# 011235813/discrete_mean_field_game

Hardware: AMD Instinct MI355X
Metric: env-steps/sec for batched d-bin population rollouts (higher is better)
Workload: dtype f32 (f64 accumulate); 1 GPU; actor_critic.train(update_every="rollout") of the drop-in class (mfg_ac2.train call surface; device-side start draw every episode, one update per 15-step rollout): d=21 topics, T=15, global batch 65536 = 65536 trajectories per GPU x 1; d=21, T=15, batch_per_gpu=65536, global_batch=65536, rng=philox4x32-10, parallelism=trajectory-sharded x1, 1 all-reduce/update

## Files before the change

### discrete_mean_field_game_amd/_lib.py

```python
from __future__ import annotations

import ctypes as C
import os
import subprocess

_HERE = os.path.dirname(os.path.abspath(__file__))
CSRC = os.path.join(_HERE, 'csrc')
LIB_PATH = os.environ.get('MFG_HIP_LIB') or os.path.join(CSRC, 'libmfg_hip.so')

MFG_MAX_D = 512
REWARD_MFG_AC2, REWARD_SYNTHETIC, REWARD_EXTERNAL = 0, 1, 2
ROLLOUT_WRITE_P, ROLLOUT_TD, ROLLOUT_DISCOUNT_POW, ROLLOUT_F64, TRAIN_APPLY = 1, 2, 4, 8, 16
PRECISION_F64, PRECISION_MIXED = 0, 1
POP_MAX_K = 65535
POP_RESIDENT_MAX_TILES = 64
STATUS_MIXED_RANGE = 1
STATUS_POP_NONFINITE = 2
ECOMM = -6
RN_TRAIN_MAX_TRAJ = 64
FORECAST_MAX_RANKS = 8
FORECAST_MAX_REPEATS = 1024
PRECISIONS = {'f64': PRECISION_F64, 'mixed': PRECISION_MIXED, 0: 0, 1: 1}


class MfgError(RuntimeError):
    code = 0


def build(force: bool = False) -> str:
    args = ['make', '-C', CSRC]
    if force:
        args.append('-B')
    subprocess.run(args, check=True, stdout=subprocess.PIPE, stderr=subprocess.STDOUT)
    return LIB_PATH


_p = C.c_void_p
_i64, _i32, _u64, _u32, _f64, _sz = C.c_int64, C.c_int, C.c_uint64, C.c_uint32, C.c_double, C.c_size_t

SIGNATURES = {
    'mfg_last_error': (C.c_char_p, []),
    'mfg_abi_version': (_i32, []),
    'mfg_set_core_mapping': (_i32, [_i32]),
    'mfg_init': (_i32, []),
    'mfg_status': (_i32, [C.POINTER(C.c_uint)]),
    'mfg_clear_status': (_i32, []),
    'mfg_ctx_create': (_i32, [C.POINTER(C.c_void_p)]),
    'mfg_ctx_destroy': (_i32, [_p]),
    'mfg_ctx_bind': (_i32, [_p]),
    'mfg_ctx_current': (_p, []),
    'mfg_ctx_status': (_i32, [_p, C.POINTER(C.c_uint)]),
    'mfg_ctx_clear_status': (_i32, [_p]),
    'mfg_ctx_adopt_comm': (_i32, [_p, _p]),
    'mfg_ctx_comm': (_p, [_p]),
    'mfg_device_info': (_i32, [C.POINTER(C.c_int), C.c_char_p, _i32]),
    'mfg_feature_index': (_i64, [_i32, _i32, _i32]),
    'mfg_num_features': (_i64, [_i32]),
    'mfg_workspace_bytes': (_sz, [_i64, _i32]),
    'mfg_gather_start': (_i32, [_p, _i64, _p, _i64, _i32, _p, _p]),
    'mfg_draw_start': (_i32, [_p, _i64, _i64, _i32, _u64, _u32, _u64, _p, _p, _p]),
    'mfg_alpha': (_i32, [_p, _i64, _i32, _p, _f64, _p, _p, _p]),
    'mfg_dirichlet_from_gamma': (_i32, [_p, _i64, _i32, _p, _p]),
    'mfg_sample_dirichlet': (_i32, [_p, _i64, _i32, _p, _f64, _f64, _u64, _u32, _u64, _i32, _p, _p]),
    'mfg_philox_raw': (_i32, [_u64, _u32, _u32, _u32, _u32, _i64, _p, _p]),
    'mfg_step_given_P': (_i32, [_p, _p, _i64, _i32, _i32, _p, _p, _p]),
    'mfg_value': (_i32, [_p, _p, _i64, _i32, _p, _p]),
    'mfg_features': (_i32, [_p, _i64, _i32, _p, _p]),
    'mfg_score': (_i32, [_p, _p, _i64, _i32, _p, _f64, _i32, _p, _p]),
    'mfg_td_pg_accumulate': (_i32, [_p, _p, _p, _p, _p, _p, _f64, _f64, _i64, _i32, _i32, _p, _p, _p, _i32, _p, _sz,
                                   _p]),
    'mfg_apply_update': (_i32, [_p, _i32, _f64, _f64, _p, _p, _p, _p]),
    'mfg_rollout': (_i32, [_p, _i64, _i32, _i32, _p, _f64, _f64, _p, _f64, _i32, _u64, _u32, _u64, _i32,
                           _p, _p, _p, _p, _p, _p, _p, _i32, _p, _sz, _p]),
    'mfg_jsd': (_i32, [_p, _p, _i64, _i32, _p, _p]),
    'mfg_grad_accumulate': (_i32, [_p, _i64, _p, _p, _p, _i64, _i32, _i32, _i32, _p, _i32, _p, _sz, _p]),
    'mfg_grad_apply': (_i32, [_p, _i64, _p, _p, _p, _i64, _i32, _i32, _i32, _p, _f64, _f64, _p, _p, _p, _p, _sz, _p]),
# ... 124 lines not shown
```

### discrete_mean_field_game_amd/csrc/mfg_grad.h

```cpp
#pragma once
#include <hip/hip_runtime.h>
#include <stdint.h>

#include "mfg_core.h"

using namespace mfg;

constexpr int MFG_GRAD_SMALL_MAX_D = 28;
constexpr int GR_OUT_PER_THREAD = 4;
constexpr int GR_OUT_PER_BLOCK = GR_OUT_PER_THREAD * BLOCK;

struct GradArgs {
  const float* pi;
  int64_t stride_b;
  const double* delta;
  const double* g;
  const float* reward;
  int64_t N;
  int T, d, chunk;
  int64_t nsb;
  double* partial;
  int add_reward;
  unsigned* counter;
  double* G;
  int accumulate, apply;
  double lr_c, lr_a;
  double *w, *theta, *reward_acc;
};

__device__ __forceinline__ void grad_partial_body(const GradArgs& a) {
  extern __shared__ __attribute__((aligned(16))) unsigned char smem_raw[];
  const int d = a.d, Q = d * (d + 1) / 2, F = Q + d + 1, FO = F + 3;
  double* dl = reinterpret_cast<double*>(smem_raw);
  float* sp = reinterpret_cast<float*>(dl + 3 * a.chunk);
  const int tid = threadIdx.x;
// ... 47 lines not shown
      } else if (kind[u] == 2) {
        for (int q = 0; q < cn; ++q) s_ += dl[3 * q];
      } else if (kind[u] == 3) {
        for (int q = 0; q < cn; ++q) s_ += dl[3 * q + 1];
      } else if (kind[u] == 4) {
        for (int q = 0; q < cn; ++q) s_ += dl[3 * q + 2];
      } else if (kind[u] == 5) {
        s_ += (double)cn;
      }
      acc[u] = s_;
    }
  }
#pragma unroll
  for (int u = 0; u < GR_OUT_PER_THREAD; ++u) {
    const int k = blockIdx.y * GR_OUT_PER_BLOCK + u * BLOCK + tid;
    if (kind[u] >= 0) a.partial[(int64_t)blockIdx.x * FO + k] = acc[u];
  }
}
#ifndef MFG_GRAD_BODIES_ONLY
__global__ __launch_bounds__(BLOCK) void k_grad_partial(GradArgs a) { grad_partial_body(a); }
#endif

#ifndef MFG_GRAD_BODIES_ONLY
__global__ void k_add_reward(double* __restrict__ delta, const float* __restrict__ reward, int64_t N) {
  for (int64_t n = blockIdx.x * (int64_t)blockDim.x + threadIdx.x; n < N; n += (int64_t)gridDim.x * blockDim.x)
    delta[n] += (double)reward[n];
}
#endif

constexpr int GS_CH = 64;
#ifndef MFG_GS_BPC
#define MFG_GS_BPC 2
#endif

template <int D>
struct GradChunk {
  static constexpr int NL = D ? D : MFG_GRAD_SMALL_MAX_D;
  float pi[NL];
  double de, dg;
  float rr;
};

template <int D, bool WIDE>
__device__ __forceinline__ void grad_chunk_load(GradChunk<D>& c, const GradArgs& a, const double* gp, const float* rp, int d,
                                                int64_t n0, int64_t b0, int s0, int lane, float invT, float inv_d) {
  const int last = (int)((a.N - 1 - n0) < (GS_CH - 1) ? (a.N - 1 - n0) : (GS_CH - 1));
  {
    const int64_t n = n0 + (lane < last ? lane : last);
    c.de = a.delta[n];
    c.dg = gp[n];
    c.rr = rp[n];
  }
  if constexpr (!WIDE) {
    const float* cb = a.pi + b0 * a.stride_b + (int64_t)s0 * d;
    const int extra = (int)(a.stride_b - (int64_t)a.T * d);
#pragma unroll
    for (int k = 0; k < GradChunk<D>::NL; ++k) {
      if (!D && k * WAVE >= GS_CH * d) {
        c.pi[k] = 0.0f;
        continue;
      }
      int e = k * WAVE + lane;
      int j = (int)(((float)e + 0.5f) * inv_d);
      if (j > last) { j = last; e = last * d; }
      const int q = (int)(((float)(s0 + j) + 0.5f) * invT);
      c.pi[k] = cb[(unsigned)(e + __mul24(q, extra))];
// ... 104 lines not shown
  __syncthreads();
  double (*red)[3][4][WAVE] = reinterpret_cast<double (*)[3][4][WAVE]>(smem);
#pragma unroll
  for (int v = 0; v < 4; ++v) {
    red[wv][0][v][lane] = c00[v];
    red[wv][1][v][lane] = c01[v];
    red[wv][2][v][lane] = c11[v];
  }
  __syncthreads();
  double* out = a.partial + (int64_t)blockIdx.x * FO;
  for (int e = tid; e < 3 * 4 * WAVE; e += BLOCK) {
    const int t = e / (4 * WAVE), v = (e / WAVE) & 3, l = e & (WAVE - 1);
    const int gi = (t == 2 ? 16 : 0) + 4 * v + (l >> 4), gj = (t == 0 ? 0 : 16) + (l & 15);
    int k = -1;
    if (gj < d) {
      if (gi <= gj) k = feat_idx(gi, gj, d);
    } else if (gj == d) {
      if (gi <= d) k = Q + gi;
    } else if (gj == d + 1) {
      if (gi == d) k = F;
    } else if (gj == d + 2) {
      if (gi == d + 1) k = F + 1;
    } else if (gj == d + 3) {
      if (gi == d + 1) k = F + 2;
    }
    if (k >= 0) {
      double tsum = red[0][t][v][l];
#pragma unroll
      for (int q = 1; q < WAVES; ++q) tsum += red[q][t][v][l];
      out[k] = tsum;
    }
  }
  if (!a.counter) return;
  __shared__ int s_last;
  __threadfence();
  __syncthreads();
  if (tid == 0) s_last = (atomicAdd(a.counter, 1u) == gridDim.x - 1) ? 1 : 0;
  __syncthreads();
  if (!s_last) return;
  __threadfence();
  double* fin = &red[0][0][0][0];
  const int nrows = (int)gridDim.x;
  for (int k = tid; k < FO; k += BLOCK) {
    double s0 = 0.0, s1 = 0.0, s2 = 0.0, s3 = 0.0;
    const double* col = a.partial + k;
    int r = 0;
    for (; r + 7 < nrows; r += 8) {
      const double v0 = col[(int64_t)r * FO], v1 = col[(int64_t)(r + 1) * FO], v2 = col[(int64_t)(r + 2) * FO],
                   v3 = col[(int64_t)(r + 3) * FO], v4 = col[(int64_t)(r + 4) * FO], v5 = col[(int64_t)(r + 5) * FO],
                   v6 = col[(int64_t)(r + 6) * FO], v7 = col[(int64_t)(r + 7) * FO];
      s0 += v0;
      s1 += v1;
      s2 += v2;
      s3 += v3;
      s0 += v4;
      s1 += v5;
      s2 += v6;
      s3 += v7;
    }
    for (; r < nrows; ++r) s0 += col[(int64_t)r * FO];
    const double tot = (s0 + s1) + (s2 + s3);
    const double gk = a.accumulate ? a.G[k] + tot : tot;
    a.G[k] = gk;
    fin[k] = gk;
  }
  __syncthreads();
  if (a.apply) {
    const double count = fin[F + 2];
    if (count > 0.0) {
      const double inv = 1.0 / count;
      for (int k = tid; k < F; k += BLOCK) a.w[k] = updated_param(a.w[k], a.lr_c, fin[k], inv);
      if (tid == 0) {
        if (a.reward_acc) *a.reward_acc += fin[F + 1] * inv;
        *a.theta = updated_param(*a.theta, a.lr_a, fin[F], inv);
      }
    }
  }
  if (tid == 0) *a.counter = 0u;
}
template <int D, bool WIDE = false>
__global__ __launch_bounds__(BLOCK) void k_grad_mfma_small(GradArgs a) { grad_mfma_small_body<D, WIDE>(a); }

constexpr int GM_KC = 32;
#ifndef MFG_GM_TPW
#define MFG_GM_TPW 8
#endif
constexpr int GM_TPW = MFG_GM_TPW;

template <int NPF>
__device__ __forceinline__ void grad_mfma_body(const GradArgs& a, int tpw) {
  extern __shared__ __attribute__((aligned(16))) unsigned char smem_raw[];
  const int d = a.d, nt = d >> 4, pitch = d + 16;
  const int Q = d * (d + 1) / 2, F = Q + d + 1, FO = F + 3;
  double* dl = reinterpret_cast<double*>(smem_raw);
  double* red = dl + GM_KC;
  float* sp = reinterpret_cast<float*>(red + 4 * BLOCK);
  const int tid = threadIdx.x, lane = tid & (WAVE - 1), wv = tid / WAVE;
  const int ntiles = nt * (nt + 1) / 2;
  const int t0 = ((int)blockIdx.y * WAVES + wv) * tpw;
  int nmine = ntiles - t0;
  nmine = nmine < 0 ? 0 : (nmine > tpw ? tpw : nmine);
  int tr[GM_TPW], tc[GM_TPW];
#pragma unroll
  for (int i = 0; i < GM_TPW; ++i) {
    int t = t0 + i, r = 0;
    if (i < nmine) {
      while (t >= nt - r) {
        t -= nt - r;
        ++r;
      }
    } else {
      t = 0;
    }
    tr[i] = r;
// ... 233 lines not shown
```

### discrete_mean_field_game_amd/csrc/mfg_kernels.hip

```cpp
#include <hip/hip_runtime.h>
#include <stdarg.h>
#include <stdint.h>
#include <stdio.h>
#include <string.h>
#include <stdlib.h>

#include <dlfcn.h>

#include <atomic>
#include <mutex>
#include <unordered_map>

#include "../../include/mfg_hip.h"
#include "mfg_core.h"
#include "mfg_evaluate_pop.h"
#include "mfg_forecast_pop.h"
#include "mfg_irl_population.h"
#include "mfg_population.h"

using namespace mfg;

static thread_local char g_err[512] = "";

static int fail(int code, const char* fmt, ...) {
// ... 1383 lines not shown

struct ApplyArgs {
  double lr_c, lr_a;
  double *w, *theta, *reward_acc;
};
static void launch_apply_update(const double* G, int d, double lr_c, double lr_a, double* w, double* theta, double* reward_acc,
                                hipStream_t st) {
  const int64_t F = mfg_num_features(d);
  hipLaunchKernelGGL(k_apply_update, dim3((unsigned)((F + 255) / 256)), dim3(256), 0, st, G, F, lr_c, lr_a, w, theta, reward_acc);
}

static bool value_batch_ok(int d) { return d > WAVE && d % 16 == 0 && d <= MFG_MAX_D; }
static size_t value_buffer_bytes(int64_t N, int d) { return value_batch_ok(d) ? (size_t)(2 * N) * 8 : 0; }

static void grad_geometry(int64_t N, int d, int* chunk, int64_t* nsb, int* nob) {
  const int64_t FO = mfg_num_features(d) + 3;
  int ch = 8192 / d;
  if (ch > 64) ch = 64;
  if (ch < 8) ch = 8;
  *chunk = ch;
  int64_t sb = (N + ch - 1) / ch;
#ifndef MFG_GRAD_WS_MB
#define MFG_GRAD_WS_MB 72
#endif
  int64_t cap = (int64_t)((long long)MFG_GRAD_WS_MB << 20) / (FO * 8);
  if (cap > 1024) cap = 1024;
  if (cap < 16) cap = 16;
  if (sb > cap) sb = cap;
  if (sb < 1) sb = 1;
  *nsb = sb;
  *nob = (int)((FO + GR_OUT_PER_BLOCK - 1) / GR_OUT_PER_BLOCK);
}

static int launch_grad(const float* pi, int64_t stride_b, const double* delta, const double* g, const float* reward,
                       int64_t N, int T, int d, double* G, int accumulate, void* ws, size_t ws_bytes, hipStream_t st,
                       const ApplyArgs* apply = nullptr, bool* applied = nullptr, bool add_reward = false,
                       const PopArgs* pop = nullptr) {
  if (applied) *applied = false;
  const int64_t FO = mfg_num_features(d) + 3;
  int chunk, nob;
  int64_t nsb;
  grad_geometry(N, d, &chunk, &nsb, &nob);
  const size_t need = (size_t)(nsb * FO * 8) + MFG_WS_CONTROL_BYTES;
  if (ws_bytes < need) return fail(MFG_EWORKSPACE, "%s: need %lld bytes, have %lld", "workspace", (long long)need,
                                   (long long)ws_bytes);
  ReduceApply rap{};
  if (apply && !accumulate) {
    rap.on = 1;
    rap.lr_c = apply->lr_c;
    rap.lr_a = apply->lr_a;
    rap.count = (double)N;
    rap.w = apply->w;
    rap.theta = apply->theta;
    rap.reward_acc = apply->reward_acc;
  }
  GradArgs a{};
  a.pi = pi;
  a.stride_b = stride_b;
  a.delta = delta;
  a.g = g;
  a.reward = reward;
  a.N = N;
  a.T = T;
  a.d = d;
  a.chunk = chunk;
  a.nsb = nsb;
  a.partial = reinterpret_cast<double*>((char*)ws + MFG_WS_CONTROL_BYTES);
  const bool small = d <= MFG_GRAD_SMALL_MAX_D;
  if (add_reward && !small)
    hipLaunchKernelGGL(k_add_reward, dim3(grid_for(N, 256, 8)), dim3(256), 0, st, const_cast<double*>(delta), reward, N);
  if (small) {
    a.add_reward = add_reward ? 1 : 0;
    const int64_t NC = (N + GS_CH - 1) / GS_CH;
    int64_t blocks = (NC + WAVES - 1) / WAVES;
    const int64_t cap = (int64_t)num_cus() * MFG_GS_BPC;
    if (blocks > cap) blocks = cap;
    if (blocks > nsb) blocks = nsb;
    if (blocks < 1) blocks = 1;
    a.nsb = blocks;
    const bool fuse = blocks <= MFG_GRAD_FUSE_MAX_ROWS;
    if (fuse) {
      a.counter = reinterpret_cast<unsigned*>(ws);
      a.G = G;
      a.accumulate = accumulate;
      if (apply) {
        a.apply = 1;
        a.lr_c = apply->lr_c;
        a.lr_a = apply->lr_a;
        a.w = apply->w;
        a.theta = apply->theta;
        a.reward_acc = apply->reward_acc;
        if (applied) *applied = true;
      }
    }
    const bool wide = stride_b - (int64_t)T * d >= (1 << 23);
    if (pop) {
      if (wide) return fail(MFG_EUNSUPPORTED, "%s", "population: trajectory stride beyond the small gradient kernel");
      launch_grad_mfma_small_pop(d == 21 || d == 15 ? d : 0, (unsigned)blocks, a, *pop, st);
      if (fuse) return check_launch("grad_mfma_small_pop");
      launch_reduce_partials_pop((unsigned)((FO + RP_OUT - 1) / RP_OUT), (const double*)a.partial, blocks, FO, G, rap, *pop, st);
      if (applied && rap.on) *applied = true;
      return check_launch("grad_mfma_small_pop");
    }
    if (wide) hipLaunchKernelGGL((k_grad_mfma_small<0, true>), dim3((unsigned)blocks), dim3(BLOCK), 0, st, a);
    else if (d == 21) hipLaunchKernelGGL((k_grad_mfma_small<21>), dim3((unsigned)blocks), dim3(BLOCK), 0, st, a);
    else if (d == 15) hipLaunchKernelGGL((k_grad_mfma_small<15>), dim3((unsigned)blocks), dim3(BLOCK), 0, st, a);
    else hipLaunchKernelGGL((k_grad_mfma_small<0>), dim3((unsigned)blocks), dim3(BLOCK), 0, st, a);
    if (fuse) return check_launch("grad_mfma_small");
    hipLaunchKernelGGL(k_reduce_partials, dim3((unsigned)((FO + RP_OUT - 1) / RP_OUT)), dim3(RP_SLICES * RP_OUT), 0, st,
                       (const double*)a.partial, blocks, FO, accumulate, G, rap);
    if (applied && rap.on) *applied = true;
    return check_launch("grad_mfma_small");
  }
  if (d % 16 == 0 && d >= 64 && d <= 4 * BLOCK) {
    const int nt = d / 16, ntiles = nt * (nt + 1) / 2;
    const int ny = (ntiles + WAVES * GM_TPW - 1) / (WAVES * GM_TPW);
    const int tpw = (ntiles + ny * WAVES - 1) / (ny * WAVES);
    a.chunk = (BLOCK % (d / 4) == 0 && (((uintptr_t)pi & 15) == 0) && (stride_b % 4 == 0)) ? 1 : 0;
    const size_t lds_m = (size_t)GM_KC * 8 + (size_t)4 * BLOCK * 8 + (size_t)GM_KC * (d + 16) * 4;
    const int npf = a.chunk ? d / 32 : 0;
    if (pop) {
      if (npf != 0 && npf != 2) return fail(MFG_EUNSUPPORTED, "%s", "population: d > 64");
      launch_grad_mfma_pop(npf, (unsigned)nsb, (unsigned)ny, lds_m, a, tpw, *pop, st);
      launch_reduce_partials_pop((unsigned)((FO + RP_OUT - 1) / RP_OUT), (const double*)a.partial, nsb, FO, G, rap, *pop, st);
      if (applied && rap.on) *applied = true;
      return check_launch("grad_mfma_pop");
    }
#ifndef MFG_GRAD_MFMA_OLD
    if (a.chunk && (d == 128 || d == 256)) {
#ifndef MFG_GM2_BPC128
#define MFG_GM2_BPC128 3
#endif
      const int64_t want = d == 256 ? (int64_t)num_cus() * 2 / Gm2Geom<256>::NY : (int64_t)num_cus() * MFG_GM2_BPC128 / Gm2Geom<128>::NY;
      if (nsb > want) nsb = want;
      a.nsb = nsb;
      if (d == 256) hipLaunchKernelGGL((k_grad_mfma2<256>), dim3((unsigned)nsb, (unsigned)Gm2Geom<256>::NY), dim3(BLOCK), lds_m, st, a);
      else hipLaunchKernelGGL((k_grad_mfma2<128>), dim3((unsigned)nsb, (unsigned)Gm2Geom<128>::NY), dim3(BLOCK), lds_m, st, a);
// ... 179 lines not shown
  ReduceApply rap{};
  if (apply && !accumulate) {
    rap.on = 1;
    rap.lr_c = apply->lr_c;
    rap.lr_a = apply->lr_a;
    rap.count = (double)B;
    rap.w = apply->w;
    rap.theta = apply->theta;
    rap.reward_acc = apply->reward_acc;
  }
  if (pop) {
    if (accumulate) return fail(MFG_EUNSUPPORTED, "%s", "population: accumulated sums");
    launch_reduce_partials_pop((unsigned)((FO + RP_OUT - 1) / RP_OUT), (const double*)((char*)ws + MFG_WS_CONTROL_BYTES), nt, FO, G,
                               rap, *pop, st);
    return check_launch("core_sums_pop");
  }
  hipLaunchKernelGGL(k_reduce_partials, dim3((unsigned)((FO + RP_OUT - 1) / RP_OUT)), dim3(RP_SLICES * RP_OUT), 0, st,
                     (const double*)((char*)ws + MFG_WS_CONTROL_BYTES), nt, FO, accumulate, G, rap);
  return check_launch("core_sums");
}

extern "C" {

const char* mfg_last_error(void) { return g_err; }
int mfg_abi_version(void) { return 18; }

int mfg_init(void) {
  if (!htab_ptr()) return fail(MFG_ELAUNCH, "%s", "mfg_init: no HIP device / table initialisation failed");
  if (!status_word().host) return fail(MFG_ELAUNCH, "%s", "mfg_init: status word allocation failed");
  return MFG_OK;
}

int mfg_set_core_mapping(int mode) { return core_mapping_set(mode); }

int mfg_status(unsigned* bits_host) {
  const StatusWord sw = status_word();
  if (!sw.host) return fail(MFG_ELAUNCH, "%s", "status word allocation failed");
  const unsigned bits = *(volatile unsigned*)sw.host;
  if (bits_host) *bits_host = bits;
  return bits ? status_error(bits) : MFG_OK;
}

int mfg_clear_status(void) {
  const StatusWord sw = status_word();
  if (!sw.host) return fail(MFG_ELAUNCH, "%s", "status word allocation failed");
  *(volatile unsigned*)sw.host = 0u;
  return MFG_OK;
}

int mfg_ctx_create(mfg_ctx_t** ctx_out) {
  REQUIRE(ctx_out, "null pointer");
  int dev = 0;
  if (hipGetDevice(&dev) != hipSuccess || dev < 0 || dev >= 64) return fail(MFG_ELAUNCH, "%s", "mfg_ctx_create: no HIP device");
  if (!htab_ptr()) return fail(MFG_ELAUNCH, "%s", "mfg_ctx_create: table initialisation failed");
  mfg_ctx* c = new (std::nothrow) mfg_ctx();
  if (!c) return fail(MFG_ELAUNCH, "%s", "mfg_ctx_create: out of memory");
  c->device = dev;
  if (!alloc_status_word(&c->sw)) {
    delete c;
    return fail(MFG_ELAUNCH, "%s", "mfg_ctx_create: status word allocation failed");
  }
  {
    std::lock_guard<std::mutex> lock(g_ctx_mu);
    g_ctx_live[c] = g_ctx_next_gen++;
  }
  *ctx_out = c;
// ... 1674 lines not shown
```

### discrete_mean_field_game_amd/csrc/mfg_population.h

```cpp
#pragma once
#include <hip/hip_runtime.h>
#include <stdint.h>

#include "mfg_core.h"

struct GradArgs;
struct ReduceApply;

namespace mfg {

struct PopArgs {
  int K;
  int L;
  int64_t F;
  int64_t s_pi0;
  int64_t s_gpi;
  int64_t s_traj;
  int64_t s_state;
  int64_t s_n;
  int64_t s_acc;
  int64_t s_ws;
  const uint64_t* seed;
  const double *shift, *alpha_scale, *lr_c, *lr_a;
  double sc, sa;
  int64_t s_P;
  int64_t s_theta_b;
  int64_t N;
  int64_t s_idx;
  int32_t* idx;
  const int32_t* state;
  unsigned* status;
};

__device__ __forceinline__ bool pop_retired(const PopArgs& p, int k) { return p.state[k] != 0; }

template <class P>
__device__ __forceinline__ P* pop_at(P* p, int64_t stride, int k) {
  return p ? p + stride * k : p;
}
template <class P>
__device__ __forceinline__ P* pop_bytes(P* p, int64_t bytes, int k) {
  using C = std::conditional_t<std::is_const_v<P>, const char, char>;
  return p ? reinterpret_cast<P*>(reinterpret_cast<C*>(p) + bytes * k) : p;
}

template <bool SUMS, int STEP, bool CTL = false>
__device__ __forceinline__ CoreArgs pop_core_args(const CoreArgs& a, const PopArgs& p, int k) {
  CoreArgs b = a;
  b.pi0 = pop_at(a.pi0, p.s_pi0, k);
  if constexpr (STEP == 0) b.theta = a.theta + k;
  else b.theta = pop_bytes(a.theta, p.s_theta_b, k);
  b.w = pop_at(a.w, p.F, k);
  b.shift = p.shift[k];
  b.alpha_scale = p.alpha_scale[k];
  b.seed = p.seed[k];
  if constexpr (CTL) b.status = p.status + k;
  b.pi_traj = pop_at(a.pi_traj, p.s_traj, k);
  b.pi_next_out = pop_at(a.pi_next_out, p.s_state, k);
  if constexpr (STEP == 0) b.reward_out = pop_at(a.reward_out, p.s_n, k);
  b.delta = pop_at(a.delta, p.s_n, k);
  b.g = pop_at(a.g, p.s_n, k);
  if constexpr (!SUMS) b.P_out = pop_at(a.P_out, p.s_P, k);
  if constexpr (SUMS) b.part_rows = pop_bytes(a.part_rows, p.s_ws, k);
  if constexpr (STEP == 2) b.pi_start_out = pop_at(a.pi_start_out, p.s_state, k);
  if constexpr (STEP == 1) {
    b.step_G = pop_at(a.step_G, p.F + 3, k);
    b.step_rows = pop_bytes(a.step_rows, p.s_ws, k);
    b.w_out = pop_at(a.w_out, p.F, k);
    b.theta_out = pop_bytes(a.theta_out, p.s_ws, k);
    b.pend_reward_acc = pop_at(a.pend_reward_acc, p.s_acc, k);
    b.pend_lr_c = p.lr_c[k] * p.sc;
    b.pend_lr_a = p.lr_a[k] * p.sa;
  }
  return b;
}

int launch_core_pop(const CoreArgs& a, const PopArgs& p, bool fast, int num_cus, hipStream_t st);
int launch_eval_rollout_pop(const CoreArgs& a, const PopArgs& p, bool fast, int num_cus, hipStream_t st);
void launch_draw_start_pop(int grid, const float* mat, int64_t num_start, int64_t B, int d, uint32_t step, uint64_t traj_offset,
                           float* out, const PopArgs& p, hipStream_t st);
void launch_grad_mfma_small_pop(int D, unsigned blocks, const GradArgs& a, const PopArgs& p, hipStream_t st);
void launch_grad_partial_pop(unsigned nsb, unsigned nob, size_t lds, const GradArgs& a, const PopArgs& p, hipStream_t st);
void launch_grad_mfma_pop(int npf, unsigned nsb, unsigned ny, size_t lds, const GradArgs& a, int tpw, const PopArgs& p,
                          hipStream_t st);
void launch_reduce_partials_pop(unsigned nob, const double* partial, int64_t nsb, int64_t FO, double* G, const ReduceApply& ap,
                                const PopArgs& p, hipStream_t st);
void launch_reduce_rows_apply_pop(const double* rows, int nrows, int64_t FO, double* G, double count, double* w,
                                  const double* theta_in, double* theta_out, double* reward_acc, const PopArgs& p, hipStream_t st);

struct PopResidentArgs {
  const float* mat_pi0;
  int64_t num_start;
  float *pi_io, *pi_scratch;
  double *theta, *w, *G;
  double* reward_acc;
  int T, episodes;
  uint32_t first_step;
  double sc[MFG_POP_RESIDENT_EPISODES], sa[MFG_POP_RESIDENT_EPISODES];
};
int launch_pop_resident(const CoreArgs& a, const PopArgs& p, const PopResidentArgs& r, bool fast, hipStream_t st);

void launch_pop_retire(const mfg_pop_control_t& c, const double* theta, const double* w, int64_t F, const double* shift, bool mixed,
                       bool after_episode, hipStream_t st);

}
```

### discrete_mean_field_game_amd/csrc/mfg_population.hip

```cpp
#include "mfg_core.h"
#define MFG_GRAD_BODIES_ONLY
#include "mfg_grad.h"
#include "mfg_population.h"

namespace mfg {

#define MFG_CORE_POP_BOUNDS __launch_bounds__(BLOCK, SUMS ? 2 : (FAST ? MFG_CORE_SMALL_WAVES : MFG_CORE_SMALL_WAVES_F64))
template <bool FAST, int D, bool SUMS, int STEP>
__global__ MFG_CORE_POP_BOUNDS void k_core_pop(CoreArgs a, PopArgs p) {
  core_small_body<true, true, FAST, D, SUMS, STEP>(pop_core_args<SUMS, STEP>(a, p, blockIdx.y));
}
template <bool FAST, int D, bool SUMS, int STEP>
__global__ MFG_CORE_POP_BOUNDS void k_core_pop_ctl(CoreArgs a, PopArgs p) {
  if (pop_retired(p, blockIdx.y)) return;
  core_small_body<true, true, FAST, D, SUMS, STEP>(pop_core_args<SUMS, STEP, true>(a, p, blockIdx.y));
}
#undef MFG_CORE_POP_BOUNDS

template <bool FAST, int D, bool SUMS, int STEP>
static void go_pop(const CoreArgs& a, const PopArgs& p, int num_cus, size_t lds, hipStream_t st) {
  const int red = STEP == 1 ? core_step_red_blocks(a.d * (a.d + 1) / 2 + a.d + 1 + 3) : 0;
  if (p.state) {
    const int grid = core_small_grid<k_core_pop_ctl<FAST, D, SUMS, STEP>>(a, lds, num_cus) + red;
    hipLaunchKernelGGL((k_core_pop_ctl<FAST, D, SUMS, STEP>), dim3((unsigned)grid, (unsigned)p.K), dim3(BLOCK), lds, st, a, p);
// ... 25 lines not shown
  if (fast) go_pop<true, D, false, 0>(a, p, num_cus, lds, st);
  else go_pop<false, D, false, 0>(a, p, num_cus, lds, st);
}

int launch_core_pop(const CoreArgs& a, const PopArgs& p, bool fast, int num_cus, hipStream_t st) {
  const int d = a.d;
  if (d > WAVE) return MFG_EUNSUPPORTED;
  const size_t lds = core_small_lds(d, a.w != nullptr, true);
  if (d == 21) dispatch_pop<21>(a, p, fast, num_cus, lds, st);
  else if (d == 15) dispatch_pop<15>(a, p, fast, num_cus, lds, st);
  else if (!a.part_rows && a.step_nrows == 0) dispatch_pop<0>(a, p, fast, num_cus, lds, st);
  else return MFG_EUNSUPPORTED;
  return MFG_OK;
}

__global__ void k_draw_start_pop(const float* __restrict__ mat, int64_t num_start, int64_t B, int d, uint32_t step,
                                 uint64_t traj_offset, float* __restrict__ out, PopArgs p) {
  const int k = blockIdx.y;
  draw_start_body(mat, num_start, B, d, p.seed[k], step, traj_offset, nullptr, out + p.s_state * k);
}
__global__ void k_draw_start_pop_ctl(const float* __restrict__ mat, int64_t num_start, int64_t B, int d, uint32_t step,
                                     uint64_t traj_offset, float* __restrict__ out, PopArgs p) {
  const int k = blockIdx.y;
  if (pop_retired(p, k)) return;
  draw_start_body(mat, num_start, B, d, p.seed[k], step, traj_offset, nullptr, out + p.s_state * k);
}

void launch_draw_start_pop(int grid, const float* mat, int64_t num_start, int64_t B, int d, uint32_t step, uint64_t traj_offset,
                           float* out, const PopArgs& p, hipStream_t st) {
  hipLaunchKernelGGL(p.state ? k_draw_start_pop_ctl : k_draw_start_pop, dim3((unsigned)grid, (unsigned)p.K), dim3(256), 0, st, mat,
                     num_start, B, d, step, traj_offset, out, p);
}

__device__ __forceinline__ void pop_rebase_grad(GradArgs& a, const PopArgs& p, int k) {
  a.pi += p.s_gpi * k;
  a.delta += p.s_n * k;
  a.g += p.s_n * k;
  a.reward = pop_at(a.reward, p.s_n, k);
  a.partial = pop_bytes(a.partial, p.s_ws, k);
  a.counter = pop_bytes(a.counter, p.s_ws, k);
  a.G = pop_at(a.G, p.F + 3, k);
  a.w = pop_at(a.w, p.F, k);
  a.theta = pop_at(a.theta, 1, k);
  a.reward_acc = pop_at(a.reward_acc, p.s_acc, k);
  a.lr_c = p.lr_c[k] * p.sc;
  a.lr_a = p.lr_a[k] * p.sa;
}

template <int D>
__global__ __launch_bounds__(BLOCK) void k_grad_mfma_small_pop(GradArgs a, PopArgs p) {
  GradArgs b = a;
  pop_rebase_grad(b, p, blockIdx.y);
  grad_mfma_small_body<D, false>(b);
}
template <int D>
__global__ __launch_bounds__(BLOCK) void k_grad_mfma_small_pop_ctl(GradArgs a, PopArgs p) {
  if (pop_retired(p, blockIdx.y)) return;
  GradArgs b = a;
  pop_rebase_grad(b, p, blockIdx.y);
  grad_mfma_small_body<D, false>(b);
}

__global__ __launch_bounds__(BLOCK) void k_grad_partial_pop(GradArgs a, PopArgs p) {
  GradArgs b = a;
  pop_rebase_grad(b, p, blockIdx.z);
  grad_partial_body(b);
}
__global__ __launch_bounds__(BLOCK) void k_grad_partial_pop_ctl(GradArgs a, PopArgs p) {
  if (pop_retired(p, blockIdx.z)) return;
  GradArgs b = a;
  pop_rebase_grad(b, p, blockIdx.z);
  grad_partial_body(b);
}

template <int NPF>
__global__ __launch_bounds__(BLOCK) void k_grad_mfma_pop(GradArgs a, int tpw, PopArgs p) {
  GradArgs b = a;
  pop_rebase_grad(b, p, blockIdx.z);
  grad_mfma_body<NPF>(b, tpw);
}
template <int NPF>
// ... 119 lines not shown
```

### include/mfg_hip.h

```cpp
#ifndef MFG_HIP_H
#define MFG_HIP_H

#include <stddef.h>
#include <stdint.h>

#ifdef __cplusplus
extern "C" {
#endif

typedef void* mfg_stream_t;

enum {
  MFG_OK = 0,
  MFG_EINVAL = -1,
  MFG_ELAUNCH = -2,
  MFG_EUNSUPPORTED = -3,
  MFG_EWORKSPACE = -4,
  MFG_ERANGE = -5,
  MFG_ECOMM = -6
};

#define MFG_MAX_D 512

#define MFG_TRAJ_ID_LIMIT (1ull << 48)

enum {
  MFG_REWARD_MFG_AC2 = 0,
  MFG_REWARD_SYNTHETIC = 1,
  MFG_REWARD_EXTERNAL = 2
};

enum { MFG_PRECISION_F64 = 0, MFG_PRECISION_MIXED = 1 };

enum {
  MFG_ROLLOUT_WRITE_P = 1,
  MFG_ROLLOUT_TD = 2,
  MFG_ROLLOUT_DISCOUNT_POW = 4,
  MFG_ROLLOUT_F64 = 8
};

const char* mfg_last_error(void);
int mfg_abi_version(void);

int mfg_set_core_mapping(int mode);

int mfg_init(void);

enum { MFG_STATUS_MIXED_RANGE = 1,
       MFG_STATUS_POP_NONFINITE = 2  };
int mfg_status(unsigned* bits_host);
int mfg_clear_status(void);

typedef struct mfg_ctx mfg_ctx_t;
int mfg_ctx_create(mfg_ctx_t** ctx_out);
int mfg_ctx_destroy(mfg_ctx_t* ctx);
int mfg_ctx_bind(mfg_ctx_t* ctx);
mfg_ctx_t* mfg_ctx_current(void);
int mfg_ctx_status(mfg_ctx_t* ctx, unsigned* bits_host);
int mfg_ctx_clear_status(mfg_ctx_t* ctx);
int mfg_ctx_adopt_comm(mfg_ctx_t* ctx, void* comm);
void* mfg_ctx_comm(mfg_ctx_t* ctx);

typedef struct mfg_pop_control {
  int32_t* state;
  unsigned* status;
  double* theta_prev;
  int32_t* episodes_run;
  const double* stop_criteria;
  int32_t K;
} mfg_pop_control_t;
int mfg_ctx_set_pop_control(mfg_ctx_t* ctx, const mfg_pop_control_t* block);

int mfg_device_info(int* cu_count_host, char* arch_host, int arch_len);

int64_t mfg_feature_index(int i, int j, int d);
int64_t mfg_num_features(int d);

// ... 260 lines not shown
```

Baseline: 1.058 billion env-steps/s.

## Add lane-per-sample gradient kernel with per-wave output roles for d=15/21

Adds a new small-d gradient kernel that gives each lane one sample of a 64-sample chunk. Output features are split across the four waves, so each wave accumulates its share of the quadratic/linear features in f64 registers instead of using the MFMA tile path. Chunks are double-buffered through LDS with a prefetch stage, and the finishing reduction is factored into a shared helper. The new kernel is selected when N is at least 245760; here N = 65536 × 15 = 983040, so it runs by default. Risks include higher register and LDS pressure, and scalar f64 FMAs replacing matrix-core work.

```diff
diff --git a/discrete_mean_field_game_amd/_lib.py b/discrete_mean_field_game_amd/_lib.py
--- a/discrete_mean_field_game_amd/_lib.py
+++ b/discrete_mean_field_game_amd/_lib.py
@@ -42,6 +42,8 @@
     'mfg_last_error': (C.c_char_p, []),
     'mfg_abi_version': (_i32, []),
     'mfg_set_core_mapping': (_i32, [_i32]),
+    'mfg_set_grad_kernel': (_i32, [_i32]),
+    'mfg_grad_lane_table': (_i32, [_i32, _i32, _p, _p, _p, _i32]),
     'mfg_init': (_i32, []),
     'mfg_status': (_i32, [C.POINTER(C.c_uint)]),
     'mfg_clear_status': (_i32, []),
diff --git a/discrete_mean_field_game_amd/csrc/mfg_grad.h b/discrete_mean_field_game_amd/csrc/mfg_grad.h
--- a/discrete_mean_field_game_amd/csrc/mfg_grad.h
+++ b/discrete_mean_field_game_amd/csrc/mfg_grad.h
@@ -1,6 +1,8 @@
 #pragma once
 #include <hip/hip_runtime.h>
 #include <stdint.h>
+
+#include <utility>
 
 #include "mfg_core.h"
 
@@ -114,6 +116,54 @@
 #ifndef MFG_GS_BPC
 #define MFG_GS_BPC 2
 #endif
+
+__device__ __forceinline__ void grad_small_finish(const GradArgs& a, double* fin, int F, int FO) {
+  const int tid = threadIdx.x;
+  __shared__ int s_last;
+  __threadfence();
+  __syncthreads();
+  if (tid == 0) s_last = (atomicAdd(a.counter, 1u) == gridDim.x - 1) ? 1 : 0;
+  __syncthreads();
+  if (!s_last) return;
+  __threadfence();
+  const int nrows = (int)gridDim.x;
+  for (int k = tid; k < FO; k += BLOCK) {
+    double s0 = 0.0, s1 = 0.0, s2 = 0.0, s3 = 0.0;
+    const double* col = a.partial + k;
+    int r = 0;
+    for (; r + 7 < nrows; r += 8) {
+      const double v0 = col[(int64_t)r * FO], v1 = col[(int64_t)(r + 1) * FO], v2 = col[(int64_t)(r + 2) * FO],
+                   v3 = col[(int64_t)(r + 3) * FO], v4 = col[(int64_t)(r + 4) * FO], v5 = col[(int64_t)(r + 5) * FO],
+                   v6 = col[(int64_t)(r + 6) * FO], v7 = col[(int64_t)(r + 7) * FO];
+      s0 += v0;
+      s1 += v1;
+      s2 += v2;
+      s3 += v3;
+      s0 += v4;
+      s1 += v5;
+      s2 += v6;
+      s3 += v7;
+    }
+    for (; r < nrows; ++r) s0 += col[(int64_t)r * FO];
+    const double tot = (s0 + s1) + (s2 + s3);
+    const double gk = a.accumulate ? a.G[k] + tot : tot;
+    a.G[k] = gk;
+    fin[k] = gk;
+  }
+  __syncthreads();
+  if (a.apply) {
+    const double count = fin[F + 2];
+    if (count > 0.0) {
+      const double inv = 1.0 / count;
+      for (int k = tid; k < F; k += BLOCK) a.w[k] = updated_param(a.w[k], a.lr_c, fin[k], inv);
+      if (tid == 0) {
+        if (a.reward_acc) *a.reward_acc += fin[F + 1] * inv;
+        *a.theta = updated_param(*a.theta, a.lr_a, fin[F], inv);
+      }
+    }
+  }
+  if (tid == 0) *a.counter = 0u;
+}
 
 template <int D>
 struct GradChunk {
@@ -284,54 +334,204 @@
     }
   }
   if (!a.counter) return;
-  __shared__ int s_last;
-  __threadfence();
-  __syncthreads();
-  if (tid == 0) s_last = (atomicAdd(a.counter, 1u) == gridDim.x - 1) ? 1 : 0;
-  __syncthreads();
-  if (!s_last) return;
-  __threadfence();
-  double* fin = &red[0][0][0][0];
-  const int nrows = (int)gridDim.x;
-  for (int k = tid; k < FO; k += BLOCK) {
-    double s0 = 0.0, s1 = 0.0, s2 = 0.0, s3 = 0.0;
-    const double* col = a.partial + k;
-    int r = 0;
-    for (; r + 7 < nrows; r += 8) {
-      const double v0 = col[(int64_t)r * FO], v1 = col[(int64_t)(r + 1) * FO], v2 = col[(int64_t)(r + 2) * FO],
-                   v3 = col[(int64_t)(r + 3) * FO], v4 = col[(int64_t)(r + 4) * FO], v5 = col[(int64_t)(r + 5) * FO],
-                   v6 = col[(int64_t)(r + 6) * FO], v7 = col[(int64_t)(r + 7) * FO];
-      s0 += v0;
-      s1 += v1;
-      s2 += v2;
-      s3 += v3;
-      s0 += v4;
-      s1 += v5;
-      s2 += v6;
-      s3 += v7;
-    }
-    for (; r < nrows; ++r) s0 += col[(int64_t)r * FO];
-    const double tot = (s0 + s1) + (s2 + s3);
-    const double gk = a.accumulate ? a.G[k] + tot : tot;
-    a.G[k] = gk;
-    fin[k] = gk;
-  }
-  __syncthreads();
-  if (a.apply) {
-    const double count = fin[F + 2];
-    if (count > 0.0) {
-      const double inv = 1.0 / count;
-      for (int k = tid; k < F; k += BLOCK) a.w[k] = updated_param(a.w[k], a.lr_c, fin[k], inv);
-      if (tid == 0) {
-        if (a.reward_acc) *a.reward_acc += fin[F + 1] * inv;
-        *a.theta = updated_param(*a.theta, a.lr_a, fin[F], inv);
-      }
-    }
-  }
-  if (tid == 0) *a.counter = 0u;
+  grad_small_finish(a, &red[0][0][0][0], F, FO);
 }
 template <int D, bool WIDE = false>
 __global__ __launch_bounds__(BLOCK) void k_grad_mfma_small(GradArgs a) { grad_mfma_small_body<D, WIDE>(a); }
+
+constexpr int GL_ROLES = WAVES;
+#ifndef MFG_GL_PF
+#define MFG_GL_PF 1
+#endif
+constexpr int GL_PF = MFG_GL_PF;
+constexpr int GL_RED_ACC = 16;
+__host__ __device__ constexpr int grad_lane_fo(int d) { return d * (d + 1) / 2 + d + 1 + 3; }
+__host__ __device__ constexpr int grad_lane_role_start(int d, int r) {
+  return r * (grad_lane_fo(d) / GL_ROLES) + (r < grad_lane_fo(d) % GL_ROLES ? r : grad_lane_fo(d) % GL_ROLES);
+}
+__host__ __device__ constexpr int grad_lane_role_count(int d, int r) {
+  return grad_lane_role_start(d, r + 1) - grad_lane_role_start(d, r);
+}
+__host__ __device__ constexpr int grad_lane_row_start(int d, int i) { return i * d - (i * (i - 1)) / 2; }
+__host__ __device__ constexpr int grad_lane_out_kind(int d, int k) {
+  const int Q = d * (d + 1) / 2;
+  return k < Q ? 0 : (k < Q + d ? 1 : 2 + (k - (Q + d)));
+}
+__host__ __device__ constexpr int grad_lane_out_row(int d, int k) {
+  const int Q = d * (d + 1) / 2;
+  if (k >= Q) return k < Q + d ? k - Q : 0;
+  int i = 0;
+  while (i + 1 < d && grad_lane_row_start(d, i + 1) <= k) ++i;
+  return i;
+}
+__host__ __device__ constexpr int grad_lane_out_col(int d, int k) {
+  const int Q = d * (d + 1) / 2;
+  if (k >= Q) return 0;
+  const int i = grad_lane_out_row(d, k);
+  return i + (k - grad_lane_row_start(d, i));
+}
+
+template <int D, int K>
+__device__ __forceinline__ void grad_lane_one(double& acc, const double (&p)[D], double de, double dg, double rr, double one) {
+  constexpr int kind = grad_lane_out_kind(D, K), i = grad_lane_out_row(D, K), j = grad_lane_out_col(D, K);
+  if constexpr (kind == 0) acc = fma(de * p[i], p[j], acc);
+  else if constexpr (kind == 1) acc = fma(de, p[i], acc);
+  else if constexpr (kind == 2) acc += de;
+  else if constexpr (kind == 3) acc = fma(de, dg, acc);
+  else if constexpr (kind == 4) acc += rr;
+  else acc += one;
+}
+template <int D, int ROLE, int NA, int... U>
+__device__ __forceinline__ void grad_lane_role(double (&acc)[NA], const double (&p)[D], double de, double dg, double rr, double one,
+                                               std::integer_sequence<int, U...>) {
+  (grad_lane_one<D, grad_lane_role_start(D, ROLE) + U>(acc[U], p, de, dg, rr, one), ...);
+}
+
+template <int D, int ROLE>
+__device__ __forceinline__ void grad_lane_wave(const GradArgs& a, double (&lpi)[2][GS_CH * D], double (&lsc)[2][3][GS_CH],
+                                               double (&red)[GL_RED_ACC][WAVE + 1], int lane) {
+  constexpr int Q = D * (D + 1) / 2, F = Q + D + 1, FO = F + 3;
+  constexpr int wv = ROLE;
+  constexpr int NA = grad_lane_role_count(D, ROLE);
+  constexpr int NLW = (D - ROLE + WAVES - 1) / WAVES;
+  const bool has_g = a.g != nullptr, has_r = a.reward != nullptr;
+  const double* gp = has_g ? a.g : a.delta;
+  const float* rp = has_r ? a.reward : a.pi;
+  const float invT = 1.0f / (float)a.T, inv_d = 1.0f / (float)D;
+  const int extra = (int)(a.stride_b - (int64_t)a.T * D);
+  const int64_t NC = (a.N + GS_CH - 1) / GS_CH;
+  const int64_t nb = gridDim.x;
+  double acc[NA];
+#pragma unroll
+  for (int u = 0; u < NA; ++u) acc[u] = 0.0;
+  float npi[GL_PF][NLW];
+  double nde[GL_PF], ndg[GL_PF];
+  float nrr[GL_PF];
+  auto fetch = [&](int st, int64_t n0, int64_t b0, int s0) {
+    const int last = (int)((a.N - 1 - n0) < (GS_CH - 1) ? (a.N - 1 - n0) : (GS_CH - 1));
+    const float* cb = a.pi + b0 * a.stride_b + (int64_t)s0 * D;
+#pragma unroll
+    for (int u = 0; u < NLW; ++u) {
+      const int k = wv + WAVES * u;
+      int e = k * WAVE + lane;
+      int j = (int)(((float)e + 0.5f) * inv_d);
+      if (j > last) { j = last; e = last * D; }
+      const int q = (int)(((float)(s0 + j) + 0.5f) * invT);
+      npi[st][u] = cb[(unsigned)(e + __mul24(q, extra))];
+    }
+    const int64_t n = n0 + (lane < last ? lane : last);
+    if constexpr (wv == 1) {
+      nde[st] = a.delta[n];
+      nrr[st] = rp[n];
+    } else if constexpr (wv == 2) {
+      ndg[st] = gp[n];
+    }
+  };
+  auto park = [&](int buf, int st, int64_t n0) {
+#pragma unroll
+    for (int u = 0; u < NLW; ++u) {
+      const int k = wv + WAVES * u;
+      lpi[buf][k * WAVE + lane] = (double)npi[st][u];
+    }
+    const bool ok = n0 + lane < a.N;
+    if constexpr (wv == 1) {
+      const double rr = (ok && has_r) ? (double)nrr[st] : 0.0;
+      double de = ok ? nde[st] : 0.0;
+      if (a.add_reward) {
+        de += rr;
+        if (ok) const_cast<double*>(a.delta)[n0 + lane] = de;
+      }
+      lsc[buf][0][lane] = de;
+      lsc[buf][2][lane] = rr;
+    } else if constexpr (wv == 2) {
+      lsc[buf][1][lane] = (ok && has_g) ? ndg[st] : 0.0;
+    }
+  };
+  const int64_t step_n = nb * GS_CH, db = step_n / a.T;
+  const int ds = (int)(step_n - db * a.T);
+  int64_t ch = blockIdx.x, nf = ch * GS_CH, b1 = nf / a.T;
+  int s1 = (int)(nf - b1 * a.T);
+  auto advance = [&]() {
+    const bool go = nf + step_n < a.N;
+    nf += go ? step_n : 0;
+    b1 += go ? db : 0;
+    s1 += go ? ds : 0;
+    const bool wrap = s1 >= a.T;
+    s1 -= wrap ? a.T : 0;
+    b1 += wrap ? 1 : 0;
+  };
+  if (ch >= NC) return;
+#pragma unroll
+  for (int st = 0; st < GL_PF; ++st) {
+    if (st) advance();
+    fetch(st, nf, b1, s1);
+  }
+  int buf = 0;
+  auto consume = [&](int st, bool refill) {
+    const int64_t n0 = ch * GS_CH;
+    park(buf, st, n0);
+    if (refill) {
+      advance();
+      fetch(st, nf, b1, s1);
+    }
+    asm volatile("s_waitcnt lgkmcnt(0)\n\ts_barrier" ::: "memory");
+    double p[D];
+    const double de = lsc[buf][0][lane], dg = lsc[buf][1][lane], rr = lsc[buf][2][lane];
+#pragma unroll
+    for (int c = 0; c < D; ++c) p[c] = lpi[buf][lane * D + c];
+    const double one = n0 + lane < a.N ? 1.0 : 0.0;
+    grad_lane_role<D, ROLE>(acc, p, de, dg, rr, one, std::make_integer_sequence<int, NA>{});
+    ch += nb;
+    buf ^= 1;
+  };
+  const int64_t nch = (NC - ch + nb - 1) / nb;
+  for (int64_t r = nch / GL_PF; r > 0; --r) {
+#pragma unroll
+    for (int st = 0; st < GL_PF; ++st) consume(st, true);
+  }
+  const int rem = (int)(nch % GL_PF);
+#pragma unroll
+  for (int st = 0; st < GL_PF - 1; ++st)
+    if (st < rem) consume(st, false);
+  double res = 0.0;
+  const int ri = lane & (GL_RED_ACC - 1), rq = lane / GL_RED_ACC;
+#pragma unroll
+  for (int p = 0; p * GL_RED_ACC < NA; ++p) {
+    asm volatile("s_waitcnt lgkmcnt(0)" ::: "memory");
+    __builtin_amdgcn_wave_barrier();
+#pragma unroll
+    for (int i = 0; i < GL_RED_ACC; ++i) red[i][lane] = p * GL_RED_ACC + i < NA ? acc[(p * GL_RED_ACC + i) % NA] : 0.0;
+    asm volatile("s_waitcnt lgkmcnt(0)" ::: "memory");
+    __builtin_amdgcn_wave_barrier();
+    double s = red[ri][GL_RED_ACC * rq];
+#pragma unroll
+    for (int j = 1; j < WAVE / 4; ++j) s += red[ri][GL_RED_ACC * rq + j];
+    s += __shfl_xor(s, 16);
+    s += __shfl_xor(s, 32);
+    res = rq == p ? s : res;
+  }
+  constexpr int start = grad_lane_role_start(D, ROLE);
+  if (lane < NA) a.partial[(int64_t)blockIdx.x * FO + start + lane] = res;
+}
+
+template <int D>
+__device__ __forceinline__ void grad_lane_body(const GradArgs& a) {
+  static_assert(GL_ROLES == 4 && WAVES == 4 && GS_CH == WAVE, "four wave roles, a lane per sample of a chunk");
+  constexpr int F = D * (D + 1) / 2 + D + 1, FO = F + 3;
+  __shared__ double lpi[2][GS_CH * D];
+  __shared__ double lsc[2][3][GS_CH];
+  __shared__ double fin[FO];
+  __shared__ double red[WAVES][GL_RED_ACC][WAVE + 1];
+  const int lane = threadIdx.x & (WAVE - 1), wv = __builtin_amdgcn_readfirstlane(threadIdx.x / WAVE);
+  if (wv == 0) grad_lane_wave<D, 0>(a, lpi, lsc, red[0], lane);
+  else if (wv == 1) grad_lane_wave<D, 1>(a, lpi, lsc, red[1], lane);
+  else if (wv == 2) grad_lane_wave<D, 2>(a, lpi, lsc, red[2], lane);
+  else grad_lane_wave<D, 3>(a, lpi, lsc, red[3], lane);
+  if (!a.counter) return;
+  grad_small_finish(a, fin, F, FO);
+}
+template <int D>
+__global__ __launch_bounds__(BLOCK, MFG_GS_BPC) void k_grad_lane(GradArgs a) { grad_lane_body<D>(a); }
 
 constexpr int GM_KC = 32;
 #ifndef MFG_GM_TPW
diff --git a/discrete_mean_field_game_amd/csrc/mfg_grad_lane_pop.hip b/discrete_mean_field_game_amd/csrc/mfg_grad_lane_pop.hip
--- /dev/null
+++ b/discrete_mean_field_game_amd/csrc/mfg_grad_lane_pop.hip
@@ -0,0 +1,28 @@
+#include "mfg_core.h"
+#define MFG_GRAD_BODIES_ONLY
+#include "mfg_grad.h"
+#include "mfg_population.h"
+
+namespace mfg {
+
+template <int D>
+__global__ __launch_bounds__(BLOCK, MFG_GS_BPC) void k_grad_lane_pop(GradArgs a, PopArgs p) {
+  GradArgs b = a;
+  pop_rebase_grad(b, p, blockIdx.y);
+  grad_lane_body<D>(b);
+}
+template <int D>
+__global__ __launch_bounds__(BLOCK, MFG_GS_BPC) void k_grad_lane_pop_ctl(GradArgs a, PopArgs p) {
+  if (pop_retired(p, blockIdx.y)) return;
+  GradArgs b = a;
+  pop_rebase_grad(b, p, blockIdx.y);
+  grad_lane_body<D>(b);
+}
+
+void launch_grad_lane_pop(int D, unsigned blocks, const GradArgs& a, const PopArgs& p, hipStream_t st) {
+  const dim3 grid(blocks, (unsigned)p.K);
+  auto* k = D == 21 ? (p.state ? k_grad_lane_pop_ctl<21> : k_grad_lane_pop<21>) : (p.state ? k_grad_lane_pop_ctl<15> : k_grad_lane_pop<15>);
+  hipLaunchKernelGGL(k, grid, dim3(BLOCK), 0, st, a, p);
+}
+
+}
diff --git a/discrete_mean_field_game_amd/csrc/mfg_kernels.hip b/discrete_mean_field_game_amd/csrc/mfg_kernels.hip
--- a/discrete_mean_field_game_amd/csrc/mfg_kernels.hip
+++ b/discrete_mean_field_game_amd/csrc/mfg_kernels.hip
@@ -1439,6 +1439,17 @@
   *nob = (int)((FO + GR_OUT_PER_BLOCK - 1) / GR_OUT_PER_BLOCK);
 }
 
+static std::atomic<int> g_grad_kernel{0};
+#ifndef MFG_GRAD_LANE_MIN_N
+#define MFG_GRAD_LANE_MIN_N 245760
+#endif
+static bool grad_lane_wanted(int64_t N, int d, bool wide) {
+  if ((d != 21 && d != 15) || wide) return false;
+  const int mode = g_grad_kernel.load();
+  if (mode) return mode == 2;
+  return N >= MFG_GRAD_LANE_MIN_N;
+}
+
 static int launch_grad(const float* pi, int64_t stride_b, const double* delta, const double* g, const float* reward,
                        int64_t N, int T, int d, double* G, int accumulate, void* ws, size_t ws_bytes, hipStream_t st,
                        const ApplyArgs* apply = nullptr, bool* applied = nullptr, bool add_reward = false,
@@ -1479,7 +1490,9 @@
   if (small) {
     a.add_reward = add_reward ? 1 : 0;
     const int64_t NC = (N + GS_CH - 1) / GS_CH;
-    int64_t blocks = (NC + WAVES - 1) / WAVES;
+    const bool wide = stride_b - (int64_t)T * d >= (1 << 23);
+    const bool lane = grad_lane_wanted(N, d, wide);
+    int64_t blocks = lane ? NC : (NC + WAVES - 1) / WAVES;
     const int64_t cap = (int64_t)num_cus() * MFG_GS_BPC;
     if (blocks > cap) blocks = cap;
     if (blocks > nsb) blocks = nsb;
@@ -1500,16 +1513,18 @@
         if (applied) *applied = true;
       }
     }
-    const bool wide = stride_b - (int64_t)T * d >= (1 << 23);
     if (pop) {
       if (wide) return fail(MFG_EUNSUPPORTED, "%s", "population: trajectory stride beyond the small gradient kernel");
-      launch_grad_mfma_small_pop(d == 21 || d == 15 ? d : 0, (unsigned)blocks, a, *pop, st);
+      if (lane) launch_grad_lane_pop(d, (unsigned)blocks, a, *pop, st);
+      else launch_grad_mfma_small_pop(d == 21 || d == 15 ? d : 0, (unsigned)blocks, a, *pop, st);
       if (fuse) return check_launch("grad_mfma_small_pop");
       launch_reduce_partials_pop((unsigned)((FO + RP_OUT - 1) / RP_OUT), (const double*)a.partial, blocks, FO, G, rap, *pop, st);
       if (applied && rap.on) *applied = true;
       return check_launch("grad_mfma_small_pop");
     }
-    if (wide) hipLaunchKernelGGL((k_grad_mfma_small<0, true>), dim3((unsigned)blocks), dim3(BLOCK), 0, st, a);
+    if (lane && d == 21) hipLaunchKernelGGL((k_grad_lane<21>), dim3((unsigned)blocks), dim3(BLOCK), 0, st, a);
+    else if (lane) hipLaunchKernelGGL((k_grad_lane<15>), dim3((unsigned)blocks), dim3(BLOCK), 0, st, a);
+    else if (wide) hipLaunchKernelGGL((k_grad_mfma_small<0, true>), dim3((unsigned)blocks), dim3(BLOCK), 0, st, a);
     else if (d == 21) hipLaunchKernelGGL((k_grad_mfma_small<21>), dim3((unsigned)blocks), dim3(BLOCK), 0, st, a);
     else if (d == 15) hipLaunchKernelGGL((k_grad_mfma_small<15>), dim3((unsigned)blocks), dim3(BLOCK), 0, st, a);
     else hipLaunchKernelGGL((k_grad_mfma_small<0>), dim3((unsigned)blocks), dim3(BLOCK), 0, st, a);
@@ -1755,6 +1770,17 @@
 }
 
 int mfg_set_core_mapping(int mode) { return core_mapping_set(mode); }
+int mfg_set_grad_kernel(int mode) { return g_grad_kernel.exchange(mode < 0 || mode > 2 ? 0 : mode); }
+int mfg_grad_lane_table(int d, int role, int* kind, int* row, int* col, int cap) {
+  if ((d != 21 && d != 15) || role < 0 || role >= GL_ROLES) return MFG_EINVAL;
+  const int start = grad_lane_role_start(d, role), n = grad_lane_role_count(d, role);
+  for (int u = 0; u < n && u < cap; ++u) {
+    if (kind) kind[u] = grad_lane_out_kind(d, start + u);
+    if (row) row[u] = grad_lane_out_row(d, start + u);
+    if (col) col[u] = grad_lane_out_col(d, start + u);
+  }
+  return n;
+}
 
 int mfg_status(unsigned* bits_host) {
   const StatusWord sw = status_word();
diff --git a/discrete_mean_field_game_amd/csrc/mfg_population.h b/discrete_mean_field_game_amd/csrc/mfg_population.h
--- a/discrete_mean_field_game_amd/csrc/mfg_population.h
+++ b/discrete_mean_field_game_amd/csrc/mfg_population.h
@@ -44,6 +44,22 @@
   return p ? reinterpret_cast<P*>(reinterpret_cast<C*>(p) + bytes * k) : p;
 }
 
+template <class GA>
+__device__ __forceinline__ void pop_rebase_grad(GA& a, const PopArgs& p, int k) {
+  a.pi += p.s_gpi * k;
+  a.delta += p.s_n * k;
+  a.g += p.s_n * k;
+  a.reward = pop_at(a.reward, p.s_n, k);
+  a.partial = pop_bytes(a.partial, p.s_ws, k);
+  a.counter = pop_bytes(a.counter, p.s_ws, k);
+  a.G = pop_at(a.G, p.F + 3, k);
+  a.w = pop_at(a.w, p.F, k);
+  a.theta = pop_at(a.theta, 1, k);
+  a.reward_acc = pop_at(a.reward_acc, p.s_acc, k);
+  a.lr_c = p.lr_c[k] * p.sc;
+  a.lr_a = p.lr_a[k] * p.sa;
+}
+
 template <bool SUMS, int STEP, bool CTL = false>
 __device__ __forceinline__ CoreArgs pop_core_args(const CoreArgs& a, const PopArgs& p, int k) {
   CoreArgs b = a;
@@ -80,6 +96,7 @@
 void launch_draw_start_pop(int grid, const float* mat, int64_t num_start, int64_t B, int d, uint32_t step, uint64_t traj_offset,
                            float* out, const PopArgs& p, hipStream_t st);
 void launch_grad_mfma_small_pop(int D, unsigned blocks, const GradArgs& a, const PopArgs& p, hipStream_t st);
+void launch_grad_lane_pop(int D, unsigned blocks, const GradArgs& a, const PopArgs& p, hipStream_t st);
 void launch_grad_partial_pop(unsigned nsb, unsigned nob, size_t lds, const GradArgs& a, const PopArgs& p, hipStream_t st);
 void launch_grad_mfma_pop(int npf, unsigned nsb, unsigned ny, size_t lds, const GradArgs& a, int tpw, const PopArgs& p,
                           hipStream_t st);
diff --git a/discrete_mean_field_game_amd/csrc/mfg_population.hip b/discrete_mean_field_game_amd/csrc/mfg_population.hip
--- a/discrete_mean_field_game_amd/csrc/mfg_population.hip
+++ b/discrete_mean_field_game_amd/csrc/mfg_population.hip
@@ -81,21 +81,6 @@
                      num_start, B, d, step, traj_offset, out, p);
 }
 
-__device__ __forceinline__ void pop_rebase_grad(GradArgs& a, const PopArgs& p, int k) {
-  a.pi += p.s_gpi * k;
-  a.delta += p.s_n * k;
-  a.g += p.s_n * k;
-  a.reward = pop_at(a.reward, p.s_n, k);
-  a.partial = pop_bytes(a.partial, p.s_ws, k);
-  a.counter = pop_bytes(a.counter, p.s_ws, k);
-  a.G = pop_at(a.G, p.F + 3, k);
-  a.w = pop_at(a.w, p.F, k);
-  a.theta = pop_at(a.theta, 1, k);
-  a.reward_acc = pop_at(a.reward_acc, p.s_acc, k);
-  a.lr_c = p.lr_c[k] * p.sc;
-  a.lr_a = p.lr_a[k] * p.sa;
-}
-
 template <int D>
 __global__ __launch_bounds__(BLOCK) void k_grad_mfma_small_pop(GradArgs a, PopArgs p) {
   GradArgs b = a;
diff --git a/include/mfg_hip.h b/include/mfg_hip.h
--- a/include/mfg_hip.h
+++ b/include/mfg_hip.h
@@ -43,6 +43,9 @@
 int mfg_abi_version(void);
 
 int mfg_set_core_mapping(int mode);
+
+int mfg_set_grad_kernel(int mode);
+int mfg_grad_lane_table(int d, int role, int* kind, int* row, int* col, int cap);
 
 int mfg_init(void);
 
```

Measured after the change: 1.066 billion env-steps/s, median of 6. No clear change (+0.8%).
